# TongtongSong/OpenEAT

Hardware: AMD Instinct MI355X
Metric: audio-frames/sec/GPU (train) + RTF (attention-rescoring decode), 12L Conformer (higher is better)
Workload: dtype f32 (storage, accumulate, softmax, norms, losses, optimizer all fp32; every matrix product is the fp32 product to within one fp32 rounding, computed as six exact bf16 x bf16 MFMA products of three-piece operand splits h+m+l = x, dropped terms < 2^-24 |a||b| - tests hold it to the exact-fp32 mode's t; 1 GPU; configs[1]: 12L Conformer d=256 (12+3+3, h=4, ff=1024, K=15, V=3246), B=32/GPU x 10 s 16 kHz wav (T=998 frames), L=30, CTC+attention joint loss, fbank+fwd+bwd+clip+Adam, dropout 0.1; global_batch=32, parallelism=dp1, hip_graph=True

## Files before the change

include/openeat_hip.h:

```cpp
#ifndef OPENEAT_HIP_H
#define OPENEAT_HIP_H

#include <stddef.h>
#include <stdint.h>

#ifdef __cplusplus
extern "C" {
#endif

const char* oe_last_error(void);
int oe_abi_version(void);

int oe_capture_unjoined_streams(void* origin, void* const* sides, int n_sides, int* unjoined_index);

int oe_stamp(long long* buf, int slot, void* stream);

enum { OE_GATHER_NONE = 0, OE_GATHER_A = 1, OE_GATHER_B = 2 };

typedef struct oe_gemm_args {
    const float* a; long lda; int a_kmajor;
    const float* b; long ldb; int b_kmajor;
    float* c; long ldc;
    int m, n, k;
    int split_k;
// ... 45 lines not shown
    float* dx; float* ws;
} oe_ln_epilogue;

typedef struct oe_ffn_args {
    const float* x; long ldx;
    const void* w1p; const float* b1;
    const void* w2p; const float* b2;
    int rows, d, ff, act, precision;
    float drop_in; unsigned long long seed_in;
    float drop_out; unsigned long long seed_out;
    const unsigned long long* seed_dev;
    float* pre_out; float* act_out;
    const float* residual; long ldr; float beta;
    float* y; long ldy;
    oe_ln_prologue ln;
    oe_lnf_prologue lnf;
} oe_ffn_args;
size_t oe_ffn_packed_bytes(int d, int ff, int precision);
int oe_ffn_supported(int d, int ff, int precision, int act);
int oe_ffn_pack_weights(const float* w1, const float* w2, int d, int ff, int precision, void* w1p, void* w2p, void* stream);
int oe_ffn_fwd(const oe_ffn_args* args, void* stream);
int oe_ffn_pack_weights_bwd(const float* w1, const float* w2, int d, int ff, int precision, void* w2t_packed, void* w1t_packed, void* stream);
int oe_ffn_bwd(const oe_ffn_args* a, void* stream);
int oe_ffn_pack_weights_table(const void* table, int n, int max_d, int max_ff, int precision, void* stream);
int oe_ffn6_config(int mode);

typedef struct oe_rowgemm_args {
    const float* x; long ldx;
    const void* wp; const float* bias;
    int rows, k, n;
    float drop_p; unsigned long long seed; const unsigned long long* seed_dev;
    const unsigned char* rowmask;
    const float* residual; long ldr; float beta;
    float* y; long ldy;
    int act; float* preact_out; const float* actgrad_in; long ld_aux;
    oe_ln_prologue ln;
    oe_lnf_prologue lnf;
    oe_ln_epilogue lne;
} oe_rowgemm_args;
int oe_rowgemm6_supported(int k, int n);
int oe_rowgemm6_form(int rows, int k, int n);
int oe_rowgemm6(const oe_rowgemm_args* args, void* stream);
int oe_rowgemm6_pack_table(const void* table, int n, long max_pieces, void* stream);

typedef struct oe_tn_problem {
    const float* a; const float* b; float* c; float* a_colsum; const float* alpha_dev;
    long lda, ldb, ldc;
    int m, n, k;
    float alpha;
    int k_chunk, gx, gy, nz, block_start, reserved;
} oe_tn_problem;
int oe_gemm_tn_grouped_plan(oe_tn_problem* problems_host, int n, int target_blocks);
int oe_gemm_tn_grouped(const oe_tn_problem* problems_dev, int n, int total_blocks, int precision, void* stream);

int oe_colsum_f32(const float* x, long ldx, int m, int n, float alpha, const float* alpha_dev,
                  float* out, int accumulate, void* stream);

int oe_layernorm_fwd_pl(const float* x, const float* gamma, const float* beta, float eps, int rows, int d,
                        const unsigned char* rowmask, int act, float* y, float* stats, void* y_planes, long plane_stride, void* stream);
int oe_layernorm_fwd(const float* x, const float* gamma, const float* beta, float eps, int rows, int d,
                     const unsigned char* rowmask, int act, float* y, float* stats, void* stream);
size_t oe_layernorm_bwd_workspace_floats(int rows, int d);
int oe_layernorm_bwd(const float* dy, const float* x, const float* gamma, const float* beta, int act,
                     const float* stats, int rows, int d, const unsigned char* rowmask, const float* add,
                     float* dx, float* dgamma, float* dbeta, float* workspace, void* stream);
int oe_layernorm_pair_fwd(const float* x, const float* gamma1, const float* beta1, float eps1, const float* gamma2, const float* beta2,
                          float eps2, int rows, int d, float* y1, float* stats1, float* y2, float* stats2, void* stream);
int oe_layernorm_pair_bwd_dx_drop(const float* dy2, const float* x, const float* gamma1, const float* beta1, const float* stats1,
                                  const float* gamma2, const float* stats2, int rows, int d, const float* add, float* dx, float* gout,
                                  float g_alpha, float g_p, unsigned long long g_seed, const unsigned long long* g_seed_dev,
                                  const unsigned char* g_rowmask, float* workspace1, float* workspace2, void* stream);
int oe_layernorm_bwd_dx(const float* dy, const float* x, const float* gamma, const float* beta, int act, const float* stats,
                        int rows, int d, const unsigned char* rowmask, const float* add, float* dx, float* workspace,
                        void* stream);
int oe_layernorm_param_reduce(const float* workspace, int rows, int d, float* dgamma, float* dbeta, void* stream);
int oe_layernorm_param_reduce_table(const long long* table, int n, int max_rows, int max_d, void* stream);
int oe_layernorm_bwd_dx_drop(const float* dy, const float* x, const float* gamma, const float* beta, int act,
                             const float* stats, int rows, int d, const unsigned char* rowmask, const float* add, float* dx,
                             float* gout, float g_alpha, float g_p, unsigned long long g_seed,
                             const unsigned long long* g_seed_dev, const unsigned char* g_rowmask, float* workspace,
                             void* stream);
int oe_layernorm_bwd_dx_drop_pl(const float* dy, const float* x, const float* gamma, const float* beta, int act,
                                const float* stats, int rows, int d, const unsigned char* rowmask, const float* add, float* dx,
                                float* gout, float g_alpha, float g_p, unsigned long long g_seed,
                                const unsigned long long* g_seed_dev, const unsigned char* g_rowmask, float* workspace,
                                void* out_planes, long plane_stride, void* stream);

size_t oe_ctc_workspace_floats(int B, int T, int Lmax);
int oe_ctc_config(int pipe_mode, int chunks);
int oe_ctc_loss_fused_stats(const float* logits, long ldv, int B, int T, int V, const int* hlens, const int* targets,
                            int Lmax, const int* tlens, float grad_scale, const float* utt_weight, float* nll, float* loss_sum,
                            float* dlogits, float* workspace, const float* row_stats, int stats_groups, void* stream);
int oe_ctc_loss_fused(const float* logits, long ldv, int B, int T, int V, const int* hlens, const int* targets,
                      int Lmax, const int* tlens, float grad_scale, const float* utt_weight, float* nll, float* loss_sum,
                      float* dlogits, float* workspace, void* stream);

int oe_ctc_greedy(const float* logits, long ldv, int B, int T, int V, const int* hlens, int eos,
                  int* frame_best, int* out_tokens, int* out_lens, void* stream);

size_t oe_ctc_align_workspace_bytes(int B, int T, int Lmax);
int oe_ctc_align(const float* logits, long ldv, int B, int T, int V, const int* hlens, const int* targets, int Lmax,
                 const int* tlens, int* frames, int* tok_start, int* tok_end, float* tok_logp, float* score, void* workspace,
                 void* stream);

typedef struct oe_attn_args {
    const float* q; long q_bstride, q_rstride;
// ... 158 lines not shown
```

openeat_amd/csrc/gemm_tn.hip:

```cpp
#include <stdlib.h>
#include "gemm_common.h"
#include "../../include/openeat_hip.h"

typedef __bf16 bf16x8 __attribute__((ext_vector_type(8)));
typedef __bf16 bf16x4 __attribute__((ext_vector_type(4)));
typedef short s16x4 __attribute__((ext_vector_type(4)));

#define TN_KROWS 32
#define TN_COLS 128
#define TN_PITCH (TN_COLS + 16)
#define TN_PLANE (TN_KROWS * TN_PITCH)
#define TN_THREADS 512

#ifdef OE_GEMM_STAMPS
static __device__ unsigned long long* tn_stamp_buf = nullptr;
extern "C" int oe_debug_set_tn_stamp_buffer(void* p) { return (int)hipMemcpyToSymbol(HIP_SYMBOL(tn_stamp_buf), &p, sizeof(p)); }
#define TN_NOW(var)                                                                          \
    do {                                                                                     \
        __builtin_amdgcn_sched_barrier(0);                                                   \
        asm volatile("s_memtime %0\n\ts_waitcnt lgkmcnt(0)" : "=s"(var) :: "memory");        \
        __builtin_amdgcn_sched_barrier(0);                                                   \
    } while (0)
#define TN_ACC(slot) do { unsigned long long t1_; TN_NOW(t1_); tn_acc[slot] += t1_ - tn_t; tn_t = t1_; } while (0)
#else
// ... 2 lines not shown
#endif

template <int TERMS> struct TFrag { bf16x8 p[oe_npl<TERMS>::N]; };

template <int TERMS>
__device__ __forceinline__ void tn_frag(const __bf16* img, int col32, int s, int lane, TFrag<TERMS>& f) {
    const int i = lane & 15, grp = lane >> 4;
    const __bf16* p = img + (16 * s + 4 * (grp >> 1) + (i >> 2)) * TN_PITCH + col32 + 16 * (grp & 1) + 4 * (i & 3);
    typedef __attribute__((address_space(3))) s16x4 lds_s16x4;
#pragma unroll
    for (int n = 0; n < oe_npl<TERMS>::N; ++n) {
        union { s16x4 h[2]; bf16x8 v; } u;
        u.h[0] = __builtin_amdgcn_ds_read_tr16_b64_v4i16((lds_s16x4*)(p + n * TN_PLANE));
        u.h[1] = __builtin_amdgcn_ds_read_tr16_b64_v4i16((lds_s16x4*)(p + n * TN_PLANE + 8 * TN_PITCH));
        f.p[n] = u.v;
    }
}

template <int TERMS>
__device__ __forceinline__ f32x16 tn_mma(const TFrag<TERMS>& a, const TFrag<TERMS>& b, f32x16 c) {
    return oe_mma_terms<TERMS>(a, b, c);
}

struct TnRegs { float4 v[2]; };
__device__ __forceinline__ void tn_load(TnRegs& t, const float* base, long ld, int k0, int k_last) {
#pragma unroll
    for (int i = 0; i < 2; ++i) {
        const int k = min(k0 + (int)(threadIdx.x >> 5) + 16 * i, k_last);
        t.v[i] = *reinterpret_cast<const float4*>(base + (long)k * ld);
    }
}
template <int TERMS>
__device__ __forceinline__ void tn_store(const TnRegs& t, __bf16* img, int k0, int k_end) {
#pragma unroll
    for (int i = 0; i < 2; ++i) {
        const int row = (int)(threadIdx.x >> 5) + 16 * i;
        const bool live = k0 + row < k_end;
        const float x[4] = {live ? t.v[i].x : 0.f, live ? t.v[i].y : 0.f, live ? t.v[i].z : 0.f, live ? t.v[i].w : 0.f};
        constexpr int NPL = oe_npl<TERMS>::N;
        bf16x4 pl[NPL];
#pragma unroll
        for (int e = 0; e < 4; ++e) {
            __bf16 q[NPL];
            oe_split_bf16<NPL>(x[e], q);
#pragma unroll
            for (int n = 0; n < NPL; ++n) pl[n][e] = q[n];
        }
        __bf16* d = img + row * TN_PITCH + 4 * (threadIdx.x & 31);
#pragma unroll
        for (int n = 0; n < NPL; ++n) *reinterpret_cast<bf16x4*>(d + n * TN_PLANE) = pl[n];
    }
}

template <int TERMS>
__device__ __forceinline__ void tn_block(const float* __restrict__ Ap, long lda, const float* __restrict__ Bp, long ldb,
                                         float* __restrict__ C, long ldc, int M, int N, int Mr, int Nr, int K, int k_chunk,
                                         int tile_x, int tile_y, int tile_z, const EpiParams& ep) {
    constexpr int NPL = oe_npl<TERMS>::N;
    constexpr int OP_ELEMS = NPL * TN_PLANE;
    constexpr int BUF_ELEMS = 2 * OP_ELEMS;
    constexpr int XCH_BYTES = 4 * 2 * 32 * 64 * 4;
    constexpr int IMG_ELEMS = (2 * BUF_ELEMS * 2 >= XCH_BYTES) ? 2 * BUF_ELEMS : XCH_BYTES / 2;
    __shared__ __attribute__((aligned(16))) __bf16 img[IMG_ELEMS];
    __shared__ float csum_s[TN_COLS];

    const int lane = threadIdx.x & 63;
    const int wave = __builtin_amdgcn_readfirstlane(threadIdx.x >> 6);
    const int grp = wave >> 2, wm = (wave >> 1) & 1, wn = wave & 1;
    const long m0 = (long)tile_y * TN_COLS, n0 = (long)tile_x * TN_COLS;
    const int k_begin = tile_z * k_chunk;
    const int k_end = min(K, k_begin + k_chunk);
    const int nchunks = (k_end - k_begin + TN_KROWS - 1) / TN_KROWS;

    const int c4 = 4 * (threadIdx.x & 31);
    const float* a_src = Ap + min(m0 + c4, (long)Mr - 4);
    const float* b_src = Bp + min(n0 + c4, (long)Nr - 4);
    const bool do_csum = ep.a_colsum != nullptr && tile_x == 0;
    float cs[4] = {0.f, 0.f, 0.f, 0.f};

    f32x16 acc[2][2];
#pragma unroll
    for (int i = 0; i < 2; ++i)
#pragma unroll
        for (int j = 0; j < 2; ++j)
#pragma unroll
            for (int r = 0; r < 16; ++r) acc[i][j][r] = 0.f;

#ifdef OE_GEMM_STAMPS
    unsigned long long tn_acc[8] = {0, 0, 0, 0, 0, 0, 0, 0}, tn_t, tn_t0;
    TN_NOW(tn_t);
    tn_t0 = tn_t;
#endif
    TnRegs ra, rb;
    if (nchunks > 0) {
        tn_load(ra, a_src, lda, k_begin, k_end - 1);
        tn_load(rb, b_src, ldb, k_begin, k_end - 1);
        if (do_csum) {
#pragma unroll
            for (int i = 0; i < 2; ++i)
                if (k_begin + (int)(threadIdx.x >> 5) + 16 * i < k_end) { cs[0] += ra.v[i].x; cs[1] += ra.v[i].y; cs[2] += ra.v[i].z; cs[3] += ra.v[i].w; }
        }
        tn_store<TERMS>(ra, img, k_begin, k_end);
        tn_store<TERMS>(rb, img + OP_ELEMS, k_begin, k_end);
    }
    __syncthreads();
    TN_ACC(0);
    for (int c = 0; c < nchunks; ++c) {
        const int kn = k_begin + (c + 1) * TN_KROWS;
        const bool more = c + 1 < nchunks;
        if (more) {
            tn_load(ra, a_src, lda, kn, k_end - 1);
            tn_load(rb, b_src, ldb, kn, k_end - 1);
        }
        TN_ACC(1);
        const __bf16* ia = img + (c & 1) * BUF_ELEMS;
        const __bf16* ib = ia + OP_ELEMS;
        TFrag<TERMS> fa[2], fb[2];
        tn_frag<TERMS>(ia, wm * 64, grp, lane, fa[0]);
        tn_frag<TERMS>(ia, wm * 64 + 32, grp, lane, fa[1]);
        tn_frag<TERMS>(ib, wn * 64, grp, lane, fb[0]);
        tn_frag<TERMS>(ib, wn * 64 + 32, grp, lane, fb[1]);
#pragma unroll
        for (int i = 0; i < 2; ++i)
#pragma unroll
            for (int j = 0; j < 2; ++j) acc[i][j] = tn_mma<TERMS>(fa[i], fb[j], acc[i][j]);
        TN_ACC(2);
#ifdef OE_GEMM_STAMPS
        asm volatile("s_waitcnt vmcnt(0)" ::: "memory");
        TN_ACC(3);
#endif
        if (more) {
            if (do_csum) {
#pragma unroll
                for (int i = 0; i < 2; ++i)
                    if (kn + (int)(threadIdx.x >> 5) + 16 * i < k_end) { cs[0] += ra.v[i].x; cs[1] += ra.v[i].y; cs[2] += ra.v[i].z; cs[3] += ra.v[i].w; }
            }
            __bf16* nx = img + ((c + 1) & 1) * BUF_ELEMS;
            tn_store<TERMS>(ra, nx, kn, k_end);
            tn_store<TERMS>(rb, nx + OP_ELEMS, kn, k_end);
        }
        TN_ACC(4);
        __syncthreads();
        TN_ACC(5);
    }

    float alpha = ep.alpha;
    if (ep.alpha_dev) alpha *= *ep.alpha_dev;

    if (do_csum) {
        if (threadIdx.x < TN_COLS) csum_s[threadIdx.x] = 0.f;
        __syncthreads();
#pragma unroll
        for (int e = 0; e < 4; ++e) {
            const float v = cs[e] + __shfl_xor(cs[e], 32, 64);
            if (lane < 32) atomicAdd(&csum_s[4 * lane + e], v);
        }
        __syncthreads();
        if (threadIdx.x < TN_COLS && m0 + threadIdx.x < M) atomicAdd(ep.a_colsum + m0 + threadIdx.x, csum_s[threadIdx.x] * alpha);
    }

    float* xch = reinterpret_cast<float*>(img);
    const int q = wave & 3;
    {
        float* mine = xch + ((q * 2 + grp) * 32) * 64 + lane;
#pragma unroll
        for (int j = 0; j < 2; ++j)
#pragma unroll
            for (int r = 0; r < 16; ++r) mine[(j * 16 + r) * 64] = grp == 0 ? acc[1][j][r] : acc[0][j][r];
    }
    __syncthreads();
    f32x16 fin[2];
    {
        const float* theirs = xch + ((q * 2 + (1 - grp)) * 32) * 64 + lane;
#pragma unroll
        for (int j = 0; j < 2; ++j)
#pragma unroll
            for (int r = 0; r < 16; ++r) fin[j][r] = (grp == 0 ? acc[0][j][r] : acc[1][j][r]) + theirs[(j * 16 + r) * 64];
    }
    const int lrow = lane & 31, lk = lane >> 5;
    const bool interior = (m0 + TN_COLS <= M) && (n0 + TN_COLS <= N);
#pragma unroll
    for (int j = 0; j < 2; ++j) {
        const long col = n0 + wn * 64 + j * 32 + lrow;
        const long row0 = m0 + wm * 64 + grp * 32 + 4 * lk;
        float* base = C + row0 * ldc + col;
#pragma unroll
        for (int r = 0; r < 16; ++r) {
            const int dr = (r & 3) + 8 * (r >> 2);
            if (!interior && !(row0 + dr < M && col < N)) continue;
            const float v = fin[j][r] * alpha;
            if (ep.atomic) atomicAdd(base + dr * ldc, v);
            else if (ep.accumulate) base[dr * ldc] += v;
            else base[dr * ldc] = v;
        }
    }
#ifdef OE_GEMM_STAMPS
    TN_ACC(6);
    if (tn_stamp_buf && threadIdx.x == 0 && blockIdx.x < 2048) {
        for (int i = 0; i < 7; ++i) tn_stamp_buf[blockIdx.x * 8 + i] = tn_acc[i];
        tn_stamp_buf[blockIdx.x * 8 + 7] = tn_t - tn_t0;
    }
#endif
}

__device__ __forceinline__ int tn_swizzle(int id, int nblk) {
    const int q = nblk >> 3, r = nblk & 7, xcd = id & 7, j = id >> 3;
    return (xcd < r ? xcd * (q + 1) : r * (q + 1) + (xcd - r) * q) + j;
}

template <int TERMS>
__global__ __launch_bounds__(TN_THREADS) void gemm_tn_planes_kernel(const float* __restrict__ Ap, long lda, const float* __restrict__ Bp, long ldb,
                                                                   float* __restrict__ C, long ldc, int M, int N, int Mr, int Nr, int K, int k_chunk,
                                                                   int gx, int gy, EpiParams ep) {
    const int swz = tn_swizzle(blockIdx.x, gridDim.x);
    tn_block<TERMS>(Ap, lda, Bp, ldb, C, ldc, M, N, Mr, Nr, K, k_chunk, swz % gx, (swz / gx) % gy, swz / (gx * gy), ep);
}

template <int TERMS>
__global__ __launch_bounds__(TN_THREADS) void gemm_tn_grouped_kernel(const oe_tn_problem* __restrict__ tab, int n_problems) {
    const int swz = tn_swizzle(blockIdx.x, gridDim.x);
    int p = 0;
    while (p + 1 < n_problems && tab[p + 1].block_start <= swz) ++p;
    const oe_tn_problem pr = tab[p];
    const int local = swz - pr.block_start;
    EpiParams ep{};
    ep.alpha = pr.alpha; ep.alpha_dev = pr.alpha_dev; ep.beta = 1.f; ep.atomic = 1; ep.a_colsum = pr.a_colsum;
    tn_block<TERMS>(pr.a, pr.lda, pr.b, pr.ldb, pr.c, pr.ldc, pr.m, pr.n, (pr.m + 3) / 4 * 4, (pr.n + 3) / 4 * 4, pr.k, pr.k_chunk,
                    local % pr.gx, (local / pr.gx) % pr.gy, local / (pr.gx * pr.gy), ep);
}

extern "C" int oe_gemm_tn_grouped_plan(oe_tn_problem* problems, int n, int target_blocks) {
    OE_REQUIRE(problems && n > 0 && target_blocks > 0, "oe_gemm_tn_grouped_plan: bad arguments");
    long tiles = 0;
    for (int i = 0; i < n; ++i) {
        oe_tn_problem& p = problems[i];
        OE_REQUIRE(p.a && p.b && p.c && p.m >= 4 && p.n >= 4 && p.k >= 1, "oe_gemm_tn_grouped_plan: problem %d: bad shape / null pointer", i);
        OE_REQUIRE((((uintptr_t)p.a | (uintptr_t)p.b) & 15) == 0 && p.lda % 4 == 0 && p.ldb % 4 == 0 && p.lda >= (p.m + 3) / 4 * 4 &&
                       p.ldb >= (p.n + 3) / 4 * 4 && p.ldc >= p.n,
                   "oe_gemm_tn_grouped_plan: problem %d: operands not 16-byte aligned / leading dimensions too short", i);
        p.gx = oe_cdiv(p.n, TN_COLS);
        p.gy = oe_cdiv(p.m, TN_COLS);
        tiles += (long)p.gx * p.gy;
    }
    const int split = (int)min(16L, max(1L, (target_blocks + tiles / 2) / tiles));
    int blocks = 0;
    for (int i = 0; i < n; ++i) {
        oe_tn_problem& p = problems[i];
        int nz = min(split, max(1, p.k / 128));
        p.k_chunk = oe_cdiv(oe_cdiv(p.k, nz), TN_KROWS) * TN_KROWS;
        p.nz = oe_cdiv(p.k, p.k_chunk);
        p.block_start = blocks;
        blocks += p.gx * p.gy * p.nz;
    }
    return blocks;
}

extern "C" int oe_gemm_tn_grouped(const oe_tn_problem* problems_dev, int n, int total_blocks, int precision, void* stream) {
    OE_REQUIRE(problems_dev && n > 0 && total_blocks > 0, "oe_gemm_tn_grouped: bad arguments");
    OE_REQUIRE(precision == 1 || precision == 3 || precision == 6, "oe_gemm_tn_grouped: precision must be 1 (bf16), 3 (bf16x3) or 6 (bf16x6)");
    if (precision == 6)
        hipLaunchKernelGGL((gemm_tn_grouped_kernel<6>), dim3(total_blocks), dim3(TN_THREADS), 0, (hipStream_t)stream, problems_dev, n);
    else if (precision == 3)
        hipLaunchKernelGGL((gemm_tn_grouped_kernel<3>), dim3(total_blocks), dim3(TN_THREADS), 0, (hipStream_t)stream, problems_dev, n);
    else
        hipLaunchKernelGGL((gemm_tn_grouped_kernel<1>), dim3(total_blocks), dim3(TN_THREADS), 0, (hipStream_t)stream, problems_dev, n);
    OE_LAUNCH_CHECK("oe_gemm_tn_grouped");
    return 0;
}

int oe_gemm_tn_planes_try(const OperandDesc& A, const OperandDesc& B, float* C, long ldc, int M, int N, int K, int sk, const EpiParams& ep,
                          int terms, hipStream_t st) {
    static const int mode = getenv("OE_GEMM_TN_PLANES") ? atoi(getenv("OE_GEMM_TN_PLANES")) : 1;
    if (!mode) return 1;
    const int Mr = (M + 3) / 4 * 4, Nr = (N + 3) / 4 * 4;
    if (!A.vec_ok || !B.vec_ok || A.ld < Mr || B.ld < Nr || M < 4 || N < 4 || K < 1) return 1;
    if (ep.bias || ep.act || ep.preact_out || ep.actgrad_in || ep.residual || ep.rowmask || ep.drop_p > 0.f || ep.beta != 1.f || ep.scatter) return 1;
    if (sk > 1 && !ep.atomic) return 1;
    const int gx = oe_cdiv(N, TN_COLS), gy = oe_cdiv(M, TN_COLS);
    if (mode == 1 && (gx * gy < 12 || K < 2048)) return 1;
    int nz = 1;
    static const int blocks_target = getenv("OE_TN_BLOCKS") ? atoi(getenv("OE_TN_BLOCKS")) : 256;
    if (ep.atomic) {
        nz = max(1, blocks_target / (gx * gy));
        nz = min(nz, max(1, K / 128));
    }
    int kc = oe_cdiv(oe_cdiv(K, nz), TN_KROWS) * TN_KROWS;
    nz = oe_cdiv(K, kc);
    if (terms == 6)
        hipLaunchKernelGGL((gemm_tn_planes_kernel<6>), dim3(gx * gy * nz), dim3(TN_THREADS), 0, st, A.p, A.ld, B.p, B.ld, C, ldc, M, N, Mr, Nr, K, kc, gx, gy, ep);
    else if (terms == 3)
        hipLaunchKernelGGL((gemm_tn_planes_kernel<3>), dim3(gx * gy * nz), dim3(TN_THREADS), 0, st, A.p, A.ld, B.p, B.ld, C, ldc, M, N, Mr, Nr, K, kc, gx, gy, ep);
    else
        hipLaunchKernelGGL((gemm_tn_planes_kernel<1>), dim3(gx * gy * nz), dim3(TN_THREADS), 0, st, A.p, A.ld, B.p, B.ld, C, ldc, M, N, Mr, Nr, K, kc, gx, gy, ep);
    OE_LAUNCH_CHECK("oe_gemm (bf16 mfma, k-major planes)");
    return 0;
}
```

openeat_amd/hip.py:

```python
from __future__ import annotations

import ctypes as C
import os
from typing import Optional

import torch

PROFILE = None

GEMM_PRECISION = int(os.environ.get("OE_GEMM_PRECISION", "0"))

_LIB_PATH = os.environ.get("OE_HIP_LIB") or os.path.join(os.path.dirname(os.path.abspath(__file__)), "lib", "libopeneat_hip.so")
_lib = None

ACT = {"none": 0, None: 0, "relu": 1, "swish": 2, "tanh": 3, "hardtanh": 4, "selu": 5, "gelu": 6}
GATHER_NONE, GATHER_A, GATHER_B = 0, 1, 2

c_fp = C.c_void_p


class GemmArgs(C.Structure):
    _fields_ = [
        ("a", c_fp), ("lda", C.c_long), ("a_kmajor", C.c_int),
        ("b", c_fp), ("ldb", C.c_long), ("b_kmajor", C.c_int),
# ... 92 lines not shown
        ("x", c_fp), ("ldx", C.c_long),
        ("wp", c_fp), ("bias", c_fp),
        ("rows", C.c_int), ("k", C.c_int), ("n", C.c_int),
        ("drop_p", C.c_float), ("seed", C.c_ulonglong), ("seed_dev", c_fp),
        ("rowmask", c_fp),
        ("residual", c_fp), ("ldr", C.c_long), ("beta", C.c_float),
        ("y", c_fp), ("ldy", C.c_long),
        ("act", C.c_int), ("preact_out", c_fp), ("actgrad_in", c_fp), ("ld_aux", C.c_long),
        ("ln", LnPrologue), ("lnf", LnfPrologue), ("lne", LnEpilogue),
    ]


class HipLibraryMissing(RuntimeError):
    pass


def lib():
    global _lib
    if _lib is None:
        if not os.path.exists(_LIB_PATH):
            raise HipLibraryMissing(
                f"{_LIB_PATH} not found - build it with `python -c 'import __graft_entry__ as g; g.build()'` "
                "(openeat_amd has no CPU fallback)")
        _lib = C.CDLL(_LIB_PATH)
        _declare(_lib)
    return _lib


def exported_symbols():
    return list(_SIGNATURES)


class TnProblem(C.Structure):
    _fields_ = [("a", C.c_void_p), ("b", C.c_void_p), ("c", C.c_void_p), ("a_colsum", C.c_void_p), ("alpha_dev", C.c_void_p),
                ("lda", C.c_long), ("ldb", C.c_long), ("ldc", C.c_long), ("m", C.c_int), ("n", C.c_int), ("k", C.c_int),
                ("alpha", C.c_float), ("k_chunk", C.c_int), ("gx", C.c_int), ("gy", C.c_int), ("nz", C.c_int),
                ("block_start", C.c_int), ("reserved", C.c_int)]


I, L, F, D, P, U64, SZ = C.c_int, C.c_long, C.c_float, C.c_double, c_fp, C.c_ulonglong, C.c_size_t
_SIGNATURES = {
    "oe_last_error": (C.c_char_p, []),
    "oe_abi_version": (I, []),
    "oe_capture_unjoined_streams": (I, [P, C.POINTER(C.c_void_p), I, C.POINTER(I)]),
    "oe_stamp": (I, [P, I, P]),
    "oe_gemm_f32": (I, [C.POINTER(GemmArgs), P]),
    "oe_split_planes": (I, [P, L, L, L, P, L, L, P]),
    "oe_gemm_pl_launches": (L, []),
    "oe_gemm_hyb_launches": (L, []),
    "oe_gemm_pl_config": (I, [I, I, I, I]),
    "oe_gemm_pl_hybrid": (I, [I]),
    "oe_gemm_tn_grouped_plan": (I, [C.POINTER(TnProblem), I, I]),
    "oe_gemm_tn_grouped": (I, [P, I, I, I, P]),
    "oe_ffn_packed_bytes": (SZ, [I, I, I]),
    "oe_ffn_supported": (I, [I, I, I, I]),
    "oe_ffn_pack_weights": (I, [P, P, I, I, I, P, P, P]),
    "oe_ffn_pack_weights_bwd": (I, [P, P, I, I, I, P, P, P]),
    "oe_ffn_pack_weights_table": (I, [P, I, I, I, I, P]),
    "oe_ffn_fwd": (I, [C.POINTER(FfnArgs), P]),
    "oe_ffn_bwd": (I, [C.POINTER(FfnArgs), P]),
    "oe_ffn6_config": (I, [I]),
    "oe_rowgemm6_supported": (I, [I, I]),
    "oe_rowgemm6": (I, [C.POINTER(RowGemmArgs), P]),
    "oe_rowgemm6_pack_table": (I, [P, I, L, P]),
    "oe_rowgemm6_form": (I, [I, I, I]),
    "oe_colsum_f32": (I, [P, L, I, I, F, P, P, I, P]),
    "oe_layernorm_fwd": (I, [P, P, P, F, I, I, P, I, P, P, P]),
    "oe_layernorm_fwd_pl": (I, [P, P, P, F, I, I, P, I, P, P, P, L, P]),
    "oe_layernorm_bwd_workspace_floats": (SZ, [I, I]),
    "oe_layernorm_pair_fwd": (I, [P, P, P, F, P, P, F, I, I, P, P, P, P, P]),
    "oe_layernorm_pair_bwd_dx_drop": (I, [P, P, P, P, P, P, P, I, I, P, P, P, F, F, U64, P, P, P, P, P]),
    "oe_layernorm_bwd": (I, [P, P, P, P, I, P, I, I, P, P, P, P, P, P, P]),
    "oe_layernorm_bwd_dx": (I, [P, P, P, P, I, P, I, I, P, P, P, P, P]),
    "oe_layernorm_param_reduce": (I, [P, I, I, P, P, P]),
    "oe_layernorm_param_reduce_table": (I, [P, I, I, I, P]),
    "oe_layernorm_bwd_dx_drop": (I, [P, P, P, P, I, P, I, I, P, P, P, P, F, F, U64, P, P, P, P]),
    "oe_layernorm_bwd_dx_drop_pl": (I, [P, P, P, P, I, P, I, I, P, P, P, P, F, F, U64, P, P, P, P, L, P]),
    "oe_ctc_workspace_floats": (SZ, [I, I, I]),
    "oe_ctc_config": (I, [I, I]),
    "oe_ctc_loss_fused": (I, [P, L, I, I, I, P, P, I, P, F, P, P, P, P, P, P]),
    "oe_ctc_loss_fused_stats": (I, [P, L, I, I, I, P, P, I, P, F, P, P, P, P, P, P, I, P]),
    "oe_ctc_greedy": (I, [P, L, I, I, I, P, I, P, P, P, P]),
    "oe_ctc_align_workspace_bytes": (SZ, [I, I, I]),
    "oe_ctc_align": (I, [P, L, I, I, I, P, P, I, P, P, P, P, P, P, P, P]),
    "oe_attention_fwd": (I, [C.POINTER(AttnArgs), P]),
    "oe_attention_bwd": (I, [C.POINTER(AttnArgs), P]),
    "oe_relpos_prepare": (I, [P, L, L, P, L, P, P, I, I, I, I, F, P, P, P]),
    "oe_relpos_backward": (I, [P, P, P, L, L, P, L, P, P, I, I, I, I, F, P, P, L, P, P, P]),
    "oe_glu_fwd": (I, [P, L, I, P, P]),
    "oe_glu_bwd": (I, [P, P, L, I, P, P]),
    "oe_dropout_scale": (I, [P, L, I, F, F, U64, P, P, P, P]),
    "oe_embed_fwd": (I, [P, P, P, L, I, I, I, F, P, P]),
    "oe_embed_bwd": (I, [P, P, L, I, I, F, P, P]),
    "oe_swap_last2": (I, [P, L, I, I, P, I, P]),
    "oe_pad1_nhwc": (I, [P, I, I, I, I, P, P]),
    "oe_pad1_nhwc_planes": (I, [P, I, I, I, I, P, P, L, P]),
    "oe_conv_dgrad_k3s2_weights": (I, [P, I, P, P]),
    "oe_axpby": (I, [P, P, L, F, F, P, P, P]),
    "oe_loss_combine": (I, [P, P, P, F, F, F, P, P]),
    "oe_loss_combine_bwd": (I, [P, F, F, F, P, P, P, P]),
    "oe_act_fwd": (I, [P, L, I, P, P]),
    "oe_act_grad": (I, [P, P, L, I, P, P]),
    "oe_log_softmax": (I, [P, L, I, P, P]),
    "oe_topk_rows": (I, [P, L, I, I, I, P, P, P]),
    "oe_logprob_gather": (I, [P, L, I, P, I, P, P, P]),
    "oe_att_inputs": (I, [P, P, I, I, I, I, I, P, P, P, P, P, P]),
# ... 106 lines not shown
        if a_planes is not None and b_planes is not None:
            g.a_planes, g.a_plane_stride = a_planes.ptr, a_planes.stride
            g.b_planes, g.b_plane_stride = b_planes.ptr, b_planes.stride
            g.planes_k_padded = int(a_kmajor and b_kmajor and getattr(a_planes, "kpad", False) and getattr(b_planes, "kpad", False))
        elif b_planes is not None and a is not None:
            g.b_planes, g.b_plane_stride = b_planes.ptr, b_planes.stride
        if c_planes is not None:
            g.c_planes, g.c_plane_stride, g.ldcp = c_planes.ptr, c_planes.stride, c_planes.ld
    if scatter is not None:
        g.out_scatter = 1
        g.sc_t1, g.sc_f1, g.sc_t2, g.sc_f2, g.sc_s = scatter
    if conv is not None:
        g.conv_t1, g.conv_f1, g.conv_t2, g.conv_f2, g.conv_c = conv[:5]
        g.conv_k, g.conv_s = (conv[5], conv[6]) if len(conv) > 5 else (0, 0)
    if PROFILE is not None:
        e0, e1 = torch.cuda.Event(enable_timing=True), torch.cuda.Event(enable_timing=True)
        e0.record()
        check(lib().oe_gemm_f32(C.byref(g), stream()), "oe_gemm_f32")
        e1.record()
        PROFILE.append((e0, e1, 2.0 * m * n * k, (m, n, k, int(a_kmajor), int(b_kmajor), int(conv_gather), int(split_k))))
        return
    check(lib().oe_gemm_f32(C.byref(g), stream()), "oe_gemm_f32")


def tn_grouped_plan(problems, target_blocks: int = 384):
    n = len(problems)
    arr = (TnProblem * n)()
    dp = lambda t: None if t is None else t.data_ptr()
    for i, q in enumerate(problems):
        dy, x, out = q["dy"], q["x"], q["out"]
        p = arr[i]
        p.a, p.b, p.c, p.a_colsum, p.alpha_dev = dy.data_ptr(), x.data_ptr(), out.data_ptr(), dp(q.get("bias_out")), dp(q.get("alpha_dev"))
        p.lda, p.ldb, p.ldc = dy.stride(0), x.stride(0), out.stride(0)
        p.m, p.n, p.k, p.alpha = dy.shape[1], x.shape[1], dy.shape[0], float(q.get("alpha", 1.0))
    total = lib().oe_gemm_tn_grouped_plan(arr, n, int(target_blocks))
    if total < 0:
        return None
    return bytes(arr), total


def tn_grouped_launch(table_dev: torch.Tensor, n: int, total_blocks: int, precision=None, flops: float = 0.0):
    if PROFILE is not None:
        e0, e1 = torch.cuda.Event(enable_timing=True), torch.cuda.Event(enable_timing=True)
        e0.record()
        check(lib().oe_gemm_tn_grouped(C.c_void_p(table_dev.data_ptr()), n, total_blocks, GEMM_PRECISION if precision is None else precision,
                                       stream()), "oe_gemm_tn_grouped")
        e1.record()
        PROFILE.append((e0, e1, flops, ("tn_grouped", n, total_blocks, 0, 1, 1, 0)))
        return
    check(lib().oe_gemm_tn_grouped(C.c_void_p(table_dev.data_ptr()), n, total_blocks, GEMM_PRECISION if precision is None else precision,
                                   stream()), "oe_gemm_tn_grouped")


def ffn_fwd(x2, w1p, b1, w2p, b2, rows, d, ff, act, *, drop_in=0.0, seed_in=0, drop_out=0.0, seed_out=0, seed_dev=None, pre_out=None,
            act_out=None, residual=None, ldr=0, beta=1.0, y=None, precision=None, lnf=None):
    a = FfnArgs()
    dp = lambda t: None if t is None else t.data_ptr()
    a.x, a.ldx = x2.data_ptr(), x2.stride(0)
    if lnf is not None:
        a.lnf.fill(lnf)
    a.w1p, a.b1, a.w2p, a.b2 = w1p.data_ptr(), dp(b1), w2p.data_ptr(), dp(b2)
    a.rows, a.d, a.ff, a.act = rows, d, ff, act
    a.precision = GEMM_PRECISION if precision is None else precision
    a.drop_in, a.seed_in, a.drop_out, a.seed_out, a.seed_dev = drop_in, seed_in, drop_out, seed_out, dp(seed_dev)
    a.pre_out, a.act_out, a.residual, a.ldr, a.beta = dp(pre_out), dp(act_out), dp(residual), ldr, beta
    a.y, a.ldy = y.data_ptr(), y.stride(0)
    if PROFILE is not None:
        e0, e1 = torch.cuda.Event(enable_timing=True), torch.cuda.Event(enable_timing=True)
        e0.record()
        check(lib().oe_ffn_fwd(C.byref(a), stream()), "oe_ffn_fwd")
        e1.record()
        PROFILE.append((e0, e1, 4.0 * rows * d * ff, ("ffn_fwd", rows, d, ff, 0, 0, 1)))
        return
    check(lib().oe_ffn_fwd(C.byref(a), stream()), "oe_ffn_fwd")


def ffn_bwd(dy2, w2tp, w1tp, rows, d, ff, act, *, drop_in=0.0, seed_in=0, seed_dev=None, pre=None, dh=None, dx=None, precision=None, ln=None):
    a = FfnArgs()
    dp = lambda t: None if t is None else t.data_ptr()
    a.x, a.ldx = dy2.data_ptr(), dy2.stride(0)
    if ln is not None:
        a.ln.fill(ln)
    a.w1p, a.b1, a.w2p, a.b2 = w2tp.data_ptr(), None, w1tp.data_ptr(), None
    a.rows, a.d, a.ff, a.act = rows, d, ff, act
    a.precision = GEMM_PRECISION if precision is None else precision
    a.drop_in, a.seed_in, a.drop_out, a.seed_out, a.seed_dev = drop_in, seed_in, 0.0, 0, dp(seed_dev)
    a.pre_out, a.act_out, a.residual, a.ldr, a.beta = pre.data_ptr(), dh.data_ptr(), None, 0, 1.0
    a.y, a.ldy = dx.data_ptr(), dx.stride(0)
    if PROFILE is not None:
        e0, e1 = torch.cuda.Event(enable_timing=True), torch.cuda.Event(enable_timing=True)
        e0.record()
        check(lib().oe_ffn_bwd(C.byref(a), stream()), "oe_ffn_bwd")
        e1.record()
        PROFILE.append((e0, e1, 4.0 * rows * d * ff, ("ffn_bwd", rows, d, ff, 0, 0, 1)))
        return
    check(lib().oe_ffn_bwd(C.byref(a), stream()), "oe_ffn_bwd")


def rowgemm6(x, wp, y, rows, k, n, *, bias=None, drop_p=0.0, seed=0, seed_dev=None, rowmask=None, residual=None, ldr=0, beta=1.0,
             act=0, preact_out=None, actgrad_in=None, ld_aux=0, ln=None, lnf=None, lne=None):
    a = RowGemmArgs()
    dp = lambda t: None if t is None else t.data_ptr()
    a.x, a.ldx, a.wp, a.bias = (0 if x is None else x.data_ptr()), (k if x is None else x.stride(0)), wp.data_ptr(), dp(bias)
    a.rows, a.k, a.n = rows, k, n
    a.drop_p, a.seed, a.seed_dev, a.rowmask = drop_p, seed, dp(seed_dev), dp(rowmask)
    a.residual, a.ldr, a.beta = dp(residual), ldr, beta
# ... 159 lines not shown
```

Measured before the change: 1.996 million audio-frames/s.

## Pipeline TN GEMM k-loop with two-deep register prefetch and interleaved split-stores

Adds a pipelined variant of the k-major TN GEMM block, enabled by default. It keeps two register stages of global loads in flight and splits and stores the next chunk's bf16 planes to LDS between the fragment reads and the MFMAs, using sched_group_barrier to interleave them. Bounds masking now runs only on the final chunk, and the column-sum reduction uses per-wave shared slots instead of LDS atomics. The aim is to hide global-load latency and split/store cost behind MFMA work, at the price of more registers (possible occupancy loss) and extra code paths.

```diff
diff --git a/include/openeat_hip.h b/include/openeat_hip.h
--- a/include/openeat_hip.h
+++ b/include/openeat_hip.h
@@ -121,6 +121,7 @@
 } oe_tn_problem;
 int oe_gemm_tn_grouped_plan(oe_tn_problem* problems_host, int n, int target_blocks);
 int oe_gemm_tn_grouped(const oe_tn_problem* problems_dev, int n, int total_blocks, int precision, void* stream);
+int oe_gemm_tn_pipeline(int on);
 
 int oe_colsum_f32(const float* x, long ldx, int m, int n, float alpha, const float* alpha_dev,
                   float* out, int accumulate, void* stream);
diff --git a/openeat_amd/csrc/gemm_tn.hip b/openeat_amd/csrc/gemm_tn.hip
--- a/openeat_amd/csrc/gemm_tn.hip
+++ b/openeat_amd/csrc/gemm_tn.hip
@@ -78,7 +78,85 @@
     }
 }
 
-template <int TERMS>
+template <int TERMS, bool LAST>
+__device__ __forceinline__ void tn_store_pk(const TnRegs& t, __bf16* img, int k0, int k_end) {
+    constexpr int NPL = oe_npl<TERMS>::N;
+#pragma unroll
+    for (int i = 0; i < 2; ++i) {
+        const int row = (int)(threadIdx.x >> 5) + 16 * i;
+        float x[4] = {t.v[i].x, t.v[i].y, t.v[i].z, t.v[i].w};
+        if constexpr (LAST) {
+            const bool live = k0 + row < k_end;
+#pragma unroll
+            for (int e = 0; e < 4; ++e) x[e] = live ? x[e] : 0.f;
+        }
+        oe_bf16x4v pl[NPL];
+        oe_split4<NPL>(x, pl);
+        __bf16* d = img + row * TN_PITCH + 4 * (threadIdx.x & 31);
+#pragma unroll
+        for (int n = 0; n < NPL; ++n) *reinterpret_cast<oe_bf16x4v*>(d + n * TN_PLANE) = pl[n];
+    }
+}
+template <bool LAST>
+__device__ __forceinline__ void tn_csum(const TnRegs& t, int k0, int k_end, float (&cs)[4]) {
+#pragma unroll
+    for (int i = 0; i < 2; ++i) {
+        bool live = true;
+        if constexpr (LAST) live = k0 + (int)(threadIdx.x >> 5) + 16 * i < k_end;
+        cs[0] += live ? t.v[i].x : 0.f; cs[1] += live ? t.v[i].y : 0.f; cs[2] += live ? t.v[i].z : 0.f; cs[3] += live ? t.v[i].w : 0.f;
+    }
+}
+
+typedef float tn_f32x4 __attribute__((ext_vector_type(4)));
+__device__ __forceinline__ void tn_load_g(TnRegs& t, const float* base, long ld, int k0, int k_last) {
+#pragma unroll
+    for (int i = 0; i < 2; ++i) {
+        const int k = min(k0 + (int)(threadIdx.x >> 5) + 16 * i, k_last);
+        const tn_f32x4 v = *(const __attribute__((address_space(1))) tn_f32x4*)(base + (long)k * ld);
+        t.v[i] = make_float4(v[0], v[1], v[2], v[3]);
+    }
+}
+struct TnSrc { const float* a; const float* b; long lda, ldb; int k_end; };
+
+template <int TERMS, bool LOAD, int SPLIT>
+__device__ __forceinline__ void tn_step(const TnSrc& src, int k0, TnRegs& la, TnRegs& lb, const TnRegs& sa, const TnRegs& sb,
+                                        const __bf16* cur, __bf16* nxt, int grp, int wm, int wn, int lane,
+                                        f32x16 (&acc)[2][2], float (&cs)[4]) {
+    constexpr int NPL = oe_npl<TERMS>::N;
+    constexpr int OP_ELEMS = NPL * TN_PLANE;
+    if constexpr (LOAD) {
+        tn_load_g(la, src.a, src.lda, k0 + 2 * TN_KROWS, src.k_end - 1);
+        tn_load_g(lb, src.b, src.ldb, k0 + 2 * TN_KROWS, src.k_end - 1);
+        __builtin_amdgcn_sched_barrier(0);
+    }
+    TFrag<TERMS> fa[2], fb[2];
+    tn_frag<TERMS>(cur, wm * 64, grp, lane, fa[0]);
+    tn_frag<TERMS>(cur, wm * 64 + 32, grp, lane, fa[1]);
+    tn_frag<TERMS>(cur + OP_ELEMS, wn * 64, grp, lane, fb[0]);
+    tn_frag<TERMS>(cur + OP_ELEMS, wn * 64 + 32, grp, lane, fb[1]);
+    if constexpr (SPLIT != 0) {
+        tn_csum<SPLIT == 2>(sa, k0 + TN_KROWS, src.k_end, cs);
+        tn_store_pk<TERMS, SPLIT == 2>(sa, nxt, k0 + TN_KROWS, src.k_end);
+        tn_store_pk<TERMS, SPLIT == 2>(sb, nxt + OP_ELEMS, k0 + TN_KROWS, src.k_end);
+    }
+#pragma unroll
+    for (int i = 0; i < 2; ++i)
+#pragma unroll
+        for (int j = 0; j < 2; ++j) acc[i][j] = tn_mma<TERMS>(fa[i], fb[j], acc[i][j]);
+    if constexpr (SPLIT != 0) {
+        constexpr int NMFMA = 4 * TERMS, NWRITE = 4 * NPL;
+        __builtin_amdgcn_sched_group_barrier(0x100, 8 * NPL, 0);
+#pragma unroll
+        for (int m = 0; m < NMFMA; ++m) {
+            __builtin_amdgcn_sched_group_barrier(0x008, 1, 0);
+            __builtin_amdgcn_sched_group_barrier(0x002, 4, 0);
+            if (m >= NMFMA - NWRITE) __builtin_amdgcn_sched_group_barrier(0x200, 1, 0);
+        }
+    }
+    __syncthreads();
+}
+
+template <int TERMS, bool PIPE>
 __device__ __forceinline__ void tn_block(const float* __restrict__ Ap, long lda, const float* __restrict__ Bp, long ldb,
                                          float* __restrict__ C, long ldc, int M, int N, int Mr, int Nr, int K, int k_chunk,
                                          int tile_x, int tile_y, int tile_z, const EpiParams& ep) {
@@ -88,7 +166,7 @@
     constexpr int XCH_BYTES = 4 * 2 * 32 * 64 * 4;
     constexpr int IMG_ELEMS = (2 * BUF_ELEMS * 2 >= XCH_BYTES) ? 2 * BUF_ELEMS : XCH_BYTES / 2;
     __shared__ __attribute__((aligned(16))) __bf16 img[IMG_ELEMS];
-    __shared__ float csum_s[TN_COLS];
+    __shared__ float csum_s[TN_THREADS / 64][TN_COLS];
 
     const int lane = threadIdx.x & 63;
     const int wave = __builtin_amdgcn_readfirstlane(threadIdx.x >> 6);
@@ -112,77 +190,116 @@
 #pragma unroll
             for (int r = 0; r < 16; ++r) acc[i][j][r] = 0.f;
 
+    if constexpr (PIPE) {
+        TnRegs ra0, rb0, ra1, rb1;
+        const TnSrc src{a_src, b_src, lda, ldb, k_end};
+        __bf16* const im0 = img;
+        __bf16* const im1 = img + BUF_ELEMS;
+        if (nchunks > 0) {
+            tn_load_g(ra0, a_src, lda, k_begin, k_end - 1);
+            tn_load_g(rb0, b_src, ldb, k_begin, k_end - 1);
+            if (nchunks > 1) {
+                tn_load_g(ra1, a_src, lda, k_begin + TN_KROWS, k_end - 1);
+                tn_load_g(rb1, b_src, ldb, k_begin + TN_KROWS, k_end - 1);
+            }
+            tn_csum<true>(ra0, k_begin, k_end, cs);
+            tn_store_pk<TERMS, true>(ra0, im0, k_begin, k_end);
+            tn_store_pk<TERMS, true>(rb0, im0 + OP_ELEMS, k_begin, k_end);
+        }
+        __syncthreads();
+        int c = 0;
+        for (; c + 4 <= nchunks; c += 2) {
+            tn_step<TERMS, true, 1>(src, k_begin + c * TN_KROWS, ra0, rb0, ra1, rb1, im0, im1, grp, wm, wn, lane, acc, cs);
+            tn_step<TERMS, true, 1>(src, k_begin + (c + 1) * TN_KROWS, ra1, rb1, ra0, rb0, im1, im0, grp, wm, wn, lane, acc, cs);
+        }
+        const int k0 = k_begin + c * TN_KROWS, rest = nchunks - c;
+        if (rest == 3) {
+            tn_step<TERMS, true, 1>(src, k0, ra0, rb0, ra1, rb1, im0, im1, grp, wm, wn, lane, acc, cs);
+            tn_step<TERMS, false, 2>(src, k0 + TN_KROWS, ra1, rb1, ra0, rb0, im1, im0, grp, wm, wn, lane, acc, cs);
+            tn_step<TERMS, false, 0>(src, k0 + 2 * TN_KROWS, ra0, rb0, ra1, rb1, im0, im1, grp, wm, wn, lane, acc, cs);
+        } else if (rest == 2) {
+            tn_step<TERMS, false, 2>(src, k0, ra0, rb0, ra1, rb1, im0, im1, grp, wm, wn, lane, acc, cs);
+            tn_step<TERMS, false, 0>(src, k0 + TN_KROWS, ra1, rb1, ra0, rb0, im1, im0, grp, wm, wn, lane, acc, cs);
+        } else if (rest == 1) {
+            tn_step<TERMS, false, 0>(src, k0, ra0, rb0, ra1, rb1, im0, im1, grp, wm, wn, lane, acc, cs);
+        }
+    } else {
 #ifdef OE_GEMM_STAMPS
-    unsigned long long tn_acc[8] = {0, 0, 0, 0, 0, 0, 0, 0}, tn_t, tn_t0;
-    TN_NOW(tn_t);
-    tn_t0 = tn_t;
+        unsigned long long tn_acc[8] = {0, 0, 0, 0, 0, 0, 0, 0}, tn_t, tn_t0;
+        TN_NOW(tn_t);
+        tn_t0 = tn_t;
 #endif
-    TnRegs ra, rb;
-    if (nchunks > 0) {
-        tn_load(ra, a_src, lda, k_begin, k_end - 1);
-        tn_load(rb, b_src, ldb, k_begin, k_end - 1);
-        if (do_csum) {
+        TnRegs ra, rb;
+        if (nchunks > 0) {
+            tn_load(ra, a_src, lda, k_begin, k_end - 1);
+            tn_load(rb, b_src, ldb, k_begin, k_end - 1);
+            if (do_csum) {
+#pragma unroll
+                for (int i = 0; i < 2; ++i)
+                    if (k_begin + (int)(threadIdx.x >> 5) + 16 * i < k_end) { cs[0] += ra.v[i].x; cs[1] += ra.v[i].y; cs[2] += ra.v[i].z; cs[3] += ra.v[i].w; }
+            }
+            tn_store<TERMS>(ra, img, k_begin, k_end);
+            tn_store<TERMS>(rb, img + OP_ELEMS, k_begin, k_end);
+        }
+        __syncthreads();
+        TN_ACC(0);
+        for (int c = 0; c < nchunks; ++c) {
+            const int kn = k_begin + (c + 1) * TN_KROWS;
+            const bool more = c + 1 < nchunks;
+            if (more) {
+                tn_load(ra, a_src, lda, kn, k_end - 1);
+                tn_load(rb, b_src, ldb, kn, k_end - 1);
+            }
+            TN_ACC(1);
+            const __bf16* ia = img + (c & 1) * BUF_ELEMS;
+            const __bf16* ib = ia + OP_ELEMS;
+            TFrag<TERMS> fa[2], fb[2];
+            tn_frag<TERMS>(ia, wm * 64, grp, lane, fa[0]);
+            tn_frag<TERMS>(ia, wm * 64 + 32, grp, lane, fa[1]);
+            tn_frag<TERMS>(ib, wn * 64, grp, lane, fb[0]);
+            tn_frag<TERMS>(ib, wn * 64 + 32, grp, lane, fb[1]);
 #pragma unroll
             for (int i = 0; i < 2; ++i)
-                if (k_begin + (int)(threadIdx.x >> 5) + 16 * i < k_end) { cs[0] += ra.v[i].x; cs[1] += ra.v[i].y; cs[2] += ra.v[i].z; cs[3] += ra.v[i].w; }
-        }
-        tn_store<TERMS>(ra, img, k_begin, k_end);
-        tn_store<TERMS>(rb, img + OP_ELEMS, k_begin, k_end);
-    }
-    __syncthreads();
-    TN_ACC(0);
-    for (int c = 0; c < nchunks; ++c) {
-        const int kn = k_begin + (c + 1) * TN_KROWS;
-        const bool more = c + 1 < nchunks;
-        if (more) {
-            tn_load(ra, a_src, lda, kn, k_end - 1);
-            tn_load(rb, b_src, ldb, kn, k_end - 1);
-        }
-        TN_ACC(1);
-        const __bf16* ia = img + (c & 1) * BUF_ELEMS;
-        const __bf16* ib = ia + OP_ELEMS;
-        TFrag<TERMS> fa[2], fb[2];
-        tn_frag<TERMS>(ia, wm * 64, grp, lane, fa[0]);
-        tn_frag<TERMS>(ia, wm * 64 + 32, grp, lane, fa[1]);
-        tn_frag<TERMS>(ib, wn * 64, grp, lane, fb[0]);
-        tn_frag<TERMS>(ib, wn * 64 + 32, grp, lane, fb[1]);
-#pragma unroll
-        for (int i = 0; i < 2; ++i)
-#pragma unroll
-            for (int j = 0; j < 2; ++j) acc[i][j] = tn_mma<TERMS>(fa[i], fb[j], acc[i][j]);
-        TN_ACC(2);
+#pragma unroll
+                for (int j = 0; j < 2; ++j) acc[i][j] = tn_mma<TERMS>(fa[i], fb[j], acc[i][j]);
+            TN_ACC(2);
 #ifdef OE_GEMM_STAMPS
-        asm volatile("s_waitcnt vmcnt(0)" ::: "memory");
-        TN_ACC(3);
+            asm volatile("s_waitcnt vmcnt(0)" ::: "memory");
+            TN_ACC(3);
 #endif
-        if (more) {
-            if (do_csum) {
-#pragma unroll
-                for (int i = 0; i < 2; ++i)
-                    if (kn + (int)(threadIdx.x >> 5) + 16 * i < k_end) { cs[0] += ra.v[i].x; cs[1] += ra.v[i].y; cs[2] += ra.v[i].z; cs[3] += ra.v[i].w; }
+            if (more) {
+                if (do_csum) {
+#pragma unroll
+                    for (int i = 0; i < 2; ++i)
+                        if (kn + (int)(threadIdx.x >> 5) + 16 * i < k_end) { cs[0] += ra.v[i].x; cs[1] += ra.v[i].y; cs[2] += ra.v[i].z; cs[3] += ra.v[i].w; }
+                }
+                __bf16* nx = img + ((c + 1) & 1) * BUF_ELEMS;
+                tn_store<TERMS>(ra, nx, kn, k_end);
+                tn_store<TERMS>(rb, nx + OP_ELEMS, kn, k_end);
             }
-            __bf16* nx = img + ((c + 1) & 1) * BUF_ELEMS;
-            tn_store<TERMS>(ra, nx, kn, k_end);
-            tn_store<TERMS>(rb, nx + OP_ELEMS, kn, k_end);
-        }
-        TN_ACC(4);
-        __syncthreads();
-        TN_ACC(5);
+            TN_ACC(4);
+            __syncthreads();
+            TN_ACC(5);
+        }
+
     }
 
     float alpha = ep.alpha;
     if (ep.alpha_dev) alpha *= *ep.alpha_dev;
 
     if (do_csum) {
-        if (threadIdx.x < TN_COLS) csum_s[threadIdx.x] = 0.f;
-        __syncthreads();
 #pragma unroll
         for (int e = 0; e < 4; ++e) {
             const float v = cs[e] + __shfl_xor(cs[e], 32, 64);
-            if (lane < 32) atomicAdd(&csum_s[4 * lane + e], v);
+            if (lane < 32) csum_s[wave][4 * lane + e] = v;
         }
         __syncthreads();
-        if (threadIdx.x < TN_COLS && m0 + threadIdx.x < M) atomicAdd(ep.a_colsum + m0 + threadIdx.x, csum_s[threadIdx.x] * alpha);
+        if (threadIdx.x < TN_COLS && m0 + threadIdx.x < M) {
+            float sum = 0.f;
+#pragma unroll
+            for (int w = 0; w < TN_THREADS / 64; ++w) sum += csum_s[w][threadIdx.x];
+            atomicAdd(ep.a_colsum + m0 + threadIdx.x, sum * alpha);
+        }
     }
 
     float* xch = reinterpret_cast<float*>(img);
@@ -234,15 +351,15 @@
     return (xcd < r ? xcd * (q + 1) : r * (q + 1) + (xcd - r) * q) + j;
 }
 
-template <int TERMS>
+template <int TERMS, bool PIPE>
 __global__ __launch_bounds__(TN_THREADS) void gemm_tn_planes_kernel(const float* __restrict__ Ap, long lda, const float* __restrict__ Bp, long ldb,
                                                                    float* __restrict__ C, long ldc, int M, int N, int Mr, int Nr, int K, int k_chunk,
                                                                    int gx, int gy, EpiParams ep) {
     const int swz = tn_swizzle(blockIdx.x, gridDim.x);
-    tn_block<TERMS>(Ap, lda, Bp, ldb, C, ldc, M, N, Mr, Nr, K, k_chunk, swz % gx, (swz / gx) % gy, swz / (gx * gy), ep);
-}
-
-template <int TERMS>
+    tn_block<TERMS, PIPE>(Ap, lda, Bp, ldb, C, ldc, M, N, Mr, Nr, K, k_chunk, swz % gx, (swz / gx) % gy, swz / (gx * gy), ep);
+}
+
+template <int TERMS, bool PIPE>
 __global__ __launch_bounds__(TN_THREADS) void gemm_tn_grouped_kernel(const oe_tn_problem* __restrict__ tab, int n_problems) {
     const int swz = tn_swizzle(blockIdx.x, gridDim.x);
     int p = 0;
@@ -251,8 +368,19 @@
     const int local = swz - pr.block_start;
     EpiParams ep{};
     ep.alpha = pr.alpha; ep.alpha_dev = pr.alpha_dev; ep.beta = 1.f; ep.atomic = 1; ep.a_colsum = pr.a_colsum;
-    tn_block<TERMS>(pr.a, pr.lda, pr.b, pr.ldb, pr.c, pr.ldc, pr.m, pr.n, (pr.m + 3) / 4 * 4, (pr.n + 3) / 4 * 4, pr.k, pr.k_chunk,
+    tn_block<TERMS, PIPE>(pr.a, pr.lda, pr.b, pr.ldb, pr.c, pr.ldc, pr.m, pr.n, (pr.m + 3) / 4 * 4, (pr.n + 3) / 4 * 4, pr.k, pr.k_chunk,
                     local % pr.gx, (local / pr.gx) % pr.gy, local / (pr.gx * pr.gy), ep);
+}
+
+#ifdef OE_GEMM_STAMPS
+static int tn_pipeline = 0;
+#else
+static int tn_pipeline = !(getenv("OE_TN_PIPE") && atoi(getenv("OE_TN_PIPE")) == 0);
+#endif
+extern "C" int oe_gemm_tn_pipeline(int on) {
+    const int prev = tn_pipeline;
+    if (on >= 0) tn_pipeline = on != 0;
+    return prev;
 }
 
 extern "C" int oe_gemm_tn_grouped_plan(oe_tn_problem* problems, int n, int target_blocks) {
@@ -284,12 +412,17 @@
 extern "C" int oe_gemm_tn_grouped(const oe_tn_problem* problems_dev, int n, int total_blocks, int precision, void* stream) {
     OE_REQUIRE(problems_dev && n > 0 && total_blocks > 0, "oe_gemm_tn_grouped: bad arguments");
     OE_REQUIRE(precision == 1 || precision == 3 || precision == 6, "oe_gemm_tn_grouped: precision must be 1 (bf16), 3 (bf16x3) or 6 (bf16x6)");
-    if (precision == 6)
-        hipLaunchKernelGGL((gemm_tn_grouped_kernel<6>), dim3(total_blocks), dim3(TN_THREADS), 0, (hipStream_t)stream, problems_dev, n);
-    else if (precision == 3)
-        hipLaunchKernelGGL((gemm_tn_grouped_kernel<3>), dim3(total_blocks), dim3(TN_THREADS), 0, (hipStream_t)stream, problems_dev, n);
-    else
-        hipLaunchKernelGGL((gemm_tn_grouped_kernel<1>), dim3(total_blocks), dim3(TN_THREADS), 0, (hipStream_t)stream, problems_dev, n);
+    const dim3 grid(total_blocks), block(TN_THREADS);
+    const hipStream_t st = (hipStream_t)stream;
+#define TN_GROUPED(T)                                                                                            \
+    do {                                                                                                         \
+        if (tn_pipeline) hipLaunchKernelGGL((gemm_tn_grouped_kernel<T, true>), grid, block, 0, st, problems_dev, n);  \
+        else hipLaunchKernelGGL((gemm_tn_grouped_kernel<T, false>), grid, block, 0, st, problems_dev, n);         \
+    } while (0)
+    if (precision == 6) TN_GROUPED(6);
+    else if (precision == 3) TN_GROUPED(3);
+    else TN_GROUPED(1);
+#undef TN_GROUPED
     OE_LAUNCH_CHECK("oe_gemm_tn_grouped");
     return 0;
 }
@@ -312,12 +445,18 @@
     }
     int kc = oe_cdiv(oe_cdiv(K, nz), TN_KROWS) * TN_KROWS;
     nz = oe_cdiv(K, kc);
-    if (terms == 6)
-        hipLaunchKernelGGL((gemm_tn_planes_kernel<6>), dim3(gx * gy * nz), dim3(TN_THREADS), 0, st, A.p, A.ld, B.p, B.ld, C, ldc, M, N, Mr, Nr, K, kc, gx, gy, ep);
-    else if (terms == 3)
-        hipLaunchKernelGGL((gemm_tn_planes_kernel<3>), dim3(gx * gy * nz), dim3(TN_THREADS), 0, st, A.p, A.ld, B.p, B.ld, C, ldc, M, N, Mr, Nr, K, kc, gx, gy, ep);
-    else
-        hipLaunchKernelGGL((gemm_tn_planes_kernel<1>), dim3(gx * gy * nz), dim3(TN_THREADS), 0, st, A.p, A.ld, B.p, B.ld, C, ldc, M, N, Mr, Nr, K, kc, gx, gy, ep);
+    const dim3 grid(gx * gy * nz), block(TN_THREADS);
+#define TN_PLANES(T)                                                                                                                        \
+    do {                                                                                                                                    \
+        if (tn_pipeline)                                                                                                                    \
+            hipLaunchKernelGGL((gemm_tn_planes_kernel<T, true>), grid, block, 0, st, A.p, A.ld, B.p, B.ld, C, ldc, M, N, Mr, Nr, K, kc, gx, gy, ep);  \
+        else                                                                                                                                \
+            hipLaunchKernelGGL((gemm_tn_planes_kernel<T, false>), grid, block, 0, st, A.p, A.ld, B.p, B.ld, C, ldc, M, N, Mr, Nr, K, kc, gx, gy, ep); \
+    } while (0)
+    if (terms == 6) TN_PLANES(6);
+    else if (terms == 3) TN_PLANES(3);
+    else TN_PLANES(1);
+#undef TN_PLANES
     OE_LAUNCH_CHECK("oe_gemm (bf16 mfma, k-major planes)");
     return 0;
 }
diff --git a/openeat_amd/hip.py b/openeat_amd/hip.py
--- a/openeat_amd/hip.py
+++ b/openeat_amd/hip.py
@@ -168,6 +168,7 @@
     "oe_gemm_pl_hybrid": (I, [I]),
     "oe_gemm_tn_grouped_plan": (I, [C.POINTER(TnProblem), I, I]),
     "oe_gemm_tn_grouped": (I, [P, I, I, I, P]),
+    "oe_gemm_tn_pipeline": (I, [I]),
     "oe_ffn_packed_bytes": (SZ, [I, I, I]),
     "oe_ffn_supported": (I, [I, I, I, I]),
     "oe_ffn_pack_weights": (I, [P, P, I, I, I, P, P, P]),
@@ -380,6 +381,10 @@
                                    stream()), "oe_gemm_tn_grouped")
 
 
+def gemm_tn_pipeline(on: int = -1) -> int:
+    return lib().oe_gemm_tn_pipeline(int(on))
+
+
 def ffn_fwd(x2, w1p, b1, w2p, b2, rows, d, ff, act, *, drop_in=0.0, seed_in=0, drop_out=0.0, seed_out=0, seed_dev=None, pre_out=None,
             act_out=None, residual=None, ldr=0, beta=1.0, y=None, precision=None, lnf=None):
     a = FfnArgs()
```

Measured after the change: 1.999 million audio-frames/s (median of 5 runs). Within noise of the previous version (+0.2%).
